# TengdaHan/DPC

Measured on AMD Instinct MI355X. Metric: clips/sec (train step, B x8x3x5xHxW), higher is better.
Workload: dtype bf16; 1 GPU; cfg2: resnet18 2d3d, img_dim 128, seq_len 5, num_seq 8, pred_step 3, batch 128/GPU, full train step (fwd+CE/top-k+bwd+all-reduce+Adam); global_batch=128, parallelism=dp1, init=reference init, random, launch=hipGraph replay, streams=2

## Files before the change

### dpc_amd/csrc/conv_wgrad_patch.hip

```cpp
#include "conv_common.h"
#include <stdlib.h>

struct WgradPatchParams {
    const void* src;
    const void* dy;
    float* part;
    int Co, Ci, dy_ld, src_ld, Kp;
    int RH, W, NF;
    int M;
    int nks, kcps;
    int ntm, ntc;
    unsigned src_bytes, dy_bytes;
    FastDiv d_cpf;
    int cpf;
    int KT, pt, T;
    FastDiv d_T;
    int dbg;
};
#ifdef DPC_WS_PROBE
#define WP_DBG(bit) (p.dbg & (bit))
#else
#define WP_DBG(bit) 0
#endif

template <int RW>
__global__ __launch_bounds__(256, 2) void wgrad_patch_kernel(WgradPatchParams p) {
    constexpr int ROWS = 64 / RW;
    constexpr int PR = ROWS + 2, PW = RW + 4;
    constexpr int NPOS = PR * PW;
    constexpr int NPB = (NPOS + 7) / 8;
    constexpr int NIB = (NPB + 3) / 4;
    constexpr int STAGE = 8192 + NPB * 1024;
    constexpr int NST = (RW == 32 && 2 * 3 * STAGE <= 160 * 1024) ? 3 : 2;
    __shared__ __attribute__((aligned(1024))) unsigned char lds[NST * STAGE];

    const int tid = threadIdx.x;
    const int lane = tid & 63;
#ifdef DPC_SIMT_EMU
    const int wv = tid >> 6;
#else
    const int wv = __builtin_amdgcn_readfirstlane(tid >> 6);
#endif
    const int wi = wv >> 1, wj = wv & 1;
    const int l31 = lane & 31, lhi = lane >> 5;
    int id = blockIdx.x;
    {
        const int nwg = gridDim.x, q = nwg >> 3, r = nwg & 7, x = id & 7;
        id = (x < r ? x * (q + 1) : r * (q + 1) + (x - r) * q) + (id >> 3);
    }
    const int tile_c = id % p.ntc; id /= p.ntc;
    const int tile_m = id % p.ntm; id /= p.ntm;
    const int kt = id % p.KT;
    const int ks = id / p.KT;
    const int nchunks = p.NF * p.cpf;
    const int c_begin = ks * p.kcps;
    const int c_end = (c_begin + p.kcps < nchunks) ? c_begin + p.kcps : nchunks;

    const BufRsrc rs_a = make_buf_rsrc(p.dy, p.dy_bytes);
    const BufRsrc rs_b = make_buf_rsrc(p.src, p.src_bytes);
    const int pl = lane >> 3;
    const int lslot = (lane & 7) ^ (2 * (pl & 3));
    unsigned a_off[2];
    int a_row[2];
    DPC_UNROLL
    for (int i = 0; i < 2; ++i) {
        const int pp = 8 * (wv + 4 * i) + pl;
        const int r = pp / RW, c = pp % RW;
        a_row[i] = c < p.W ? r : (1 << 28);
        a_off[i] = (unsigned)((r * p.W + c) * p.dy_ld + tile_m * 64 + lslot * 8) * 2u;
    }
    unsigned b_off[NIB];
    int b_row[NIB];
    DPC_UNROLL
    for (int i = 0; i < NIB; ++i) {
        const int pp = 8 * (wv + 4 * i) + pl;
        const int prow = pp / PW, pcol = pp % PW;
        const bool ok = pp < NPOS && pcol >= 1 && pcol <= p.W;
        b_row[i] = ok ? prow - 1 : (1 << 28);
        b_off[i] = (unsigned)(((prow - 1) * p.W + (pcol - 1)) * p.src_ld + tile_c * 64 + lslot * 8) * 2u;
    }

    f32x16 acc[9];
    DPC_UNROLL
    for (int t = 0; t < 9; ++t)
        DPC_UNROLL
        for (int r = 0; r < 16; ++r) acc[t][r] = 0.f;

    constexpr int NPC = 2 + NIB;
    unsigned dma_v[NPC];
    unsigned char* dma_stage = lds;
    auto dma_prep = [&](int chunk, int buf, bool real) {
        dma_stage = lds + buf * STAGE;
        const unsigned frame = fdiv((unsigned)chunk, p.d_cpf);
        const int h0 = (chunk - (int)frame * p.cpf) * ROWS;
        const unsigned a_base = (unsigned)(((int)frame * p.RH + h0) * p.W) * (unsigned)p.dy_ld * 2u;
        const unsigned b_base = (unsigned)((((int)frame + kt - p.pt) * p.RH + h0) * p.W) * (unsigned)p.src_ld * 2u;
        DPC_UNROLL
        for (int i = 0; i < 2; ++i) {
            const bool ok = (unsigned)(h0 + a_row[i]) < (unsigned)p.RH;
            dma_v[i] = ok && real ? a_base + a_off[i] : DPC_BUF_OOB;
        }
        DPC_UNROLL
        for (int i = 0; i < NIB; ++i) {
            const bool ok = (unsigned)(h0 + b_row[i]) < (unsigned)p.RH;
            dma_v[2 + i] = ok && real ? b_base + b_off[i] : DPC_BUF_OOB;
        }
    };
    auto dma_piece = [&](auto Ic) {
        constexpr int I = decltype(Ic)::value;
        if (WP_DBG(1)) return;
        if constexpr (I < 2) {
            glds16_buf(rs_a, dma_v[I], 0u, dma_stage + (wv + 4 * I) * 1024, lane);
        } else {
            if constexpr (4 * (I - 2) + 3 < NPB) {
                glds16_buf(rs_b, dma_v[I], 0u, dma_stage + 8192 + (wv + 4 * (I - 2)) * 1024, lane);
            } else {
                if (wv + 4 * (I - 2) < NPB) glds16_buf(rs_b, dma_v[I], 0u, dma_stage + 8192 + (wv + 4 * (I - 2)) * 1024, lane);
            }
        }
    };
    auto issue = [&](int chunk, int buf) {
        dma_prep(chunk, buf, true);
        static_for<NPC>([&](auto Ic) { dma_piece(Ic); });
    };

    const int gq = lane >> 4, s16 = lane & 15, ph = s16 >> 2;
    const int lin = ((gq >> 1) * 8 + ph) * 128;
    auto slot_off = [&](int c0, int phase) {
        const int colb = (c0 + (gq & 1) * 16 + 4 * (s16 & 3)) * 2;
        return ((((colb >> 4) ^ (2 * (phase & 3))) & 7) << 4) + (colb & 15);
    };
    const int fa = lin + slot_off(wi * 32, ph);
    const int linb = ((((gq >> 1) * 8) / RW) * PW + ((gq >> 1) * 8) % RW + ph) * 128;
    int fb[3];
    DPC_UNROLL
    for (int kw = 0; kw < 3; ++kw) fb[kw] = 8192 + linb + slot_off(wj * 32, ph + kw);

#ifdef DPC_SIMT_EMU
    auto compute = [&](int buf) {
        static_for<NPC>([&](auto Ic) { dma_piece(Ic); });
        const unsigned char* st = lds + buf * STAGE;
        DPC_UNROLL
        for (int kk = 0; kk < 4; ++kk) {
            const u32x2 a0 = lds_read_tr16(st + fa + (kk * 16) * 128);
            const u32x2 a1 = lds_read_tr16(st + fa + (kk * 16 + 4) * 128);
            const u32x4 av = {a0[0], a0[1], a1[0], a1[1]};
            const int r = (kk * 16) / RW, w0 = (kk * 16) % RW;
            DPC_UNROLL
            for (int kh = 0; kh < 3; ++kh)
                DPC_UNROLL
                for (int kw = 0; kw < 3; ++kw) {
                    const int pos = (r + kh) * PW + w0 + kw;
                    const u32x2 b0 = lds_read_tr16(st + fb[kw] + pos * 128);
                    const u32x2 b1 = lds_read_tr16(st + fb[kw] + (pos + 4) * 128);
                    const u32x4 bv = {b0[0], b0[1], b1[0], b1[1]};
                    acc[kh * 3 + kw] = mfma_32x32x16_bf16(av, bv, acc[kh * 3 + kw]);
                }
        }
    };
#else
    constexpr int LOOKAHEAD = 4, RB = 8;
    const uint32_t lds0 = (uint32_t)(uintptr_t)(__attribute__((address_space(3))) unsigned char*)lds;
    auto compute = [&](int buf) {
        const uint32_t sa = lds0 + buf * STAGE + fa;
        uint32_t sb[3];
        DPC_UNROLL
        for (int kw = 0; kw < 3; ++kw) sb[kw] = lds0 + buf * STAGE + fb[kw];
        u32x2 alo[2], ahi[2], blo[RB], bhi[RB];
        auto load = [&](auto Ic) {
            constexpr int I = decltype(Ic)::value;
            constexpr int kk = I / 10, r10 = I % 10;
            if constexpr (r10 == 0) {
                asm volatile("ds_read_b64_tr_b16 %0, %1 offset:%2" : "=v"(alo[kk & 1]) : "v"(sa), "n"((kk * 16) * 128) : "memory");
                __builtin_amdgcn_sched_barrier(0);
                asm volatile("ds_read_b64_tr_b16 %0, %1 offset:%2" : "=v"(ahi[kk & 1]) : "v"(sa), "n"((kk * 16 + 4) * 128) : "memory");
                __builtin_amdgcn_sched_barrier(0);
            } else {
                constexpr int tap = r10 - 1, kh = tap / 3, kw = tap % 3, j = 9 * kk + tap;
                constexpr int pos = ((kk * 16) / RW + kh) * PW + (kk * 16) % RW + kw;
                asm volatile("ds_read_b64_tr_b16 %0, %1 offset:%2" : "=v"(blo[j % RB]) : "v"(sb[kw]), "n"(pos * 128) : "memory");
                __builtin_amdgcn_sched_barrier(0);
                asm volatile("ds_read_b64_tr_b16 %0, %1 offset:%2" : "=v"(bhi[j % RB]) : "v"(sb[kw]), "n"((pos + 4) * 128) : "memory");
                __builtin_amdgcn_sched_barrier(0);
            }
        };
        __builtin_amdgcn_sched_barrier(0);
        static_for<36>([&](auto Mc) {
            constexpr int m = decltype(Mc)::value;
            constexpr int kk = m / 9, tap = m % 9, idx = 10 * kk + 1 + tap;
            constexpr int f_prev = m == 0 ? 0 : ((idx - 1 + (tap == 0 ? -1 : 0)) + 1 + LOOKAHEAD < 40 ? (idx - 1 + (tap == 0 ? -1 : 0)) + 1 + LOOKAHEAD : 40);
            constexpr int f_now = idx + 1 + LOOKAHEAD < 40 ? idx + 1 + LOOKAHEAD : 40;
            static_for<f_now - f_prev>([&](auto Dc) { load(std::integral_constant<int, f_prev + decltype(Dc)::value>{}); });
            asm volatile("s_waitcnt lgkmcnt(%0)" ::"n"(2 * (f_now - idx - 1)) : "memory");
            __builtin_amdgcn_sched_barrier(0);
            const u32x4 av = {alo[kk & 1][0], alo[kk & 1][1], ahi[kk & 1][0], ahi[kk & 1][1]};
            const u32x4 bv = {blo[m % RB][0], blo[m % RB][1], bhi[m % RB][0], bhi[m % RB][1]};
            acc[tap] = mfma_32x32x16_bf16(av, bv, acc[tap]);
            __builtin_amdgcn_sched_barrier(0);
            if constexpr (m % 4 == 1 && m / 4 < NPC) {
                dma_piece(std::integral_constant<int, m / 4>{});
                __builtin_amdgcn_sched_barrier(0);
            }
        });
    };
#endif

    auto next_valid = [&](int c) {
        if (p.KT == 1) return c;
        while (c < c_end) {
            const unsigned frame = fdiv((unsigned)c, p.d_cpf);
            const int t = (int)frame - (int)fdiv(frame, p.d_T) * p.T;
            if ((unsigned)(t + kt - p.pt) < (unsigned)p.T) break;
            ++c;
        }
        return c;
    };
    int n_mine = 2;
    DPC_UNROLL
    for (int i = 0; i < NIB; ++i) n_mine += (wv + 4 * i < NPB) ? 1 : 0;
    int cur = next_valid(c_begin), buf = 0;
    if (NST == 3) {
        int nxt = c_end;
        if (cur < c_end) {
            issue(cur, 0);
            nxt = next_valid(cur + 1);
            if (nxt < c_end) issue(nxt, 1);
        }
        while (cur < c_end) {
            if (nxt < c_end) wait_vmcnt_upto(n_mine); else wait_vmcnt<0>();
            if (!WP_DBG(4)) barrier_lds_only();
            const int nxt2 = nxt < c_end ? next_valid(nxt + 1) : c_end;
            dma_prep(nxt2 < c_end ? nxt2 : cur, buf >= 1 ? buf - 1 : 2, nxt2 < c_end);
            if (!WP_DBG(2)) compute(buf);
            else static_for<NPC>([&](auto Ic) { dma_piece(Ic); });
            cur = nxt;
            nxt = nxt2;
            buf = buf == 2 ? 0 : buf + 1;
        }
    } else {
        if (cur < c_end) issue(cur, 0);
        __syncthreads();
        while (cur < c_end) {
            const int nxt = next_valid(cur + 1);
            dma_prep(nxt < c_end ? nxt : cur, buf ^ 1, nxt < c_end);
            if (!WP_DBG(2)) compute(buf);
            else static_for<NPC>([&](auto Ic) { dma_piece(Ic); });
            __syncthreads();
            cur = nxt;
            buf ^= 1;
        }
    }

    const int ci = tile_c * 64 + wj * 32 + l31;
    DPC_UNROLL
    for (int t = 0; t < 9; ++t)
        DPC_UNROLL
        for (int r = 0; r < 16; ++r) {
            const int co = tile_m * 64 + wi * 32 + (r & 3) + 8 * (r >> 2) + 4 * lhi;
            p.part[((long long)ks * p.Co + co) * p.Kp + (kt * 9 + t) * p.Ci + ci] = acc[t][r];
        }
}

static int wgrad_patch_enabled() {
    static int v = -1;
    if (v < 0) {
        const char* e = getenv("DPC_WGRAD_PATCH");
        v = (e && e[0] == '0') ? 0 : 1;
    }
    return v;
}

int dpc_wgrad_patch_try(const dpc_conv_desc* d, const void* src, const void* dy, int dy_ld, float* part, int32_t* nsplit,
                        hipStream_t stream) {
    if (!wgrad_patch_enabled()) return 1;
    if (d->dtype_in != DPC_BF16 || d->mode != 0) return 1;
    if (d->KH != 3 || d->KW != 3 || d->st != 1 || d->sh != 1 || d->sw != 1 || d->ph != 1 || d->pw != 1) return 1;
    if (!((d->KT == 1 && d->pt == 0) || (d->KT == 3 && d->pt == 1))) return 1;
    if (d->RT != d->ST || d->RH != d->SH || d->RW != d->SW) return 1;
    if (d->RW > 64) return 1;
    if (d->Ci % 64 || d->Co % 64 || d->src_ld % 8 || dy_ld % 8 || dy_ld < d->Co) return 1;
    const int rwp = d->RW <= 8 ? 8 : d->RW <= 16 ? 16 : d->RW <= 32 ? 32 : 64;
    const int rows = 64 / rwp;
    if (d->RH * d->RW * 10 < ((d->RH + rows - 1) / rows) * 64 * 6) return 1;
    const long long M = (long long)d->N * d->RT * d->RH * d->RW;
    const long long sb = M * d->src_ld * 2, db = M * dy_ld * 2;
    if (sb >= (1ll << 31) || db >= (1ll << 31)) return 1;
    WgradPatchParams p;
    p.Co = d->Co; p.Ci = d->Ci; p.dy_ld = dy_ld; p.src_ld = d->src_ld; p.Kp = 9 * d->KT * d->Ci;
    p.KT = d->KT; p.pt = d->pt; p.T = d->RT; p.d_T = make_fastdiv((uint32_t)d->RT);
    p.RH = d->RH; p.W = d->RW; p.NF = d->N * d->RT; p.M = (int)M;
    p.ntm = d->Co / 64; p.ntc = d->Ci / 64;
    p.src_bytes = (unsigned)sb; p.dy_bytes = (unsigned)db;
    p.cpf = (d->RH + rows - 1) / rows;
    p.d_cpf = make_fastdiv((uint32_t)p.cpf);
    const int nchunks = p.NF * p.cpf;
    static const int target_blocks = getenv("DPC_WGRAD_PATCH_BLOCKS") ? atoi(getenv("DPC_WGRAD_PATCH_BLOCKS")) : 512;
    int want = target_blocks / (p.ntm * p.ntc * p.KT);
    if (want < 1) want = 1;
    if (want > nchunks) want = nchunks;
    p.kcps = (nchunks + want - 1) / want;
    p.nks = (nchunks + p.kcps - 1) / p.kcps;
    if (nsplit) *nsplit = p.nks;
    if (!part) return DPC_OK;
    if (!src || !dy) return DPC_ERR_ARG;
    if (((uintptr_t)src % 16) || ((uintptr_t)dy % 16)) return DPC_ERR_UNSUPPORTED;
    p.src = src; p.dy = dy; p.part = part;
#ifdef DPC_WS_PROBE
    p.dbg = getenv("DPC_WS_DBG") ? atoi(getenv("DPC_WS_DBG")) : 0;
#else
    p.dbg = 0;
#endif
    dim3 grid((unsigned)(p.ntm * p.ntc * p.KT * p.nks)), block(256);
    if (rwp == 64) {
        DPC_LAUNCH((wgrad_patch_kernel<64>), grid, block, stream, p);
    } else if (rwp == 32) {
        DPC_LAUNCH((wgrad_patch_kernel<32>), grid, block, stream, p);
    } else if (rwp == 8) {
        DPC_LAUNCH((wgrad_patch_kernel<8>), grid, block, stream, p);
    } else {
        DPC_LAUNCH((wgrad_patch_kernel<16>), grid, block, stream, p);
    }
    return dpc_launch_status();
}
```

Before: 5023 clips/s.

## Repartition wgrad patch MFMA work across waves by tap to cut LDS B reads

Each wave previously owned one 32-row Co half and all nine taps, so every wave read all nine B tap fragments from LDS per k-step. Now a wave pair splits the taps: each wave loads both A halves and five B tap slots (the centre tap is shared), reusing each B fragment for two MFMAs. This cuts the LDS transposed reads per MFMA. The block index decode is also reordered so that kt varies fastest, which changes which workgroups run close together and how they share cache. Register pressure rises from holding two A fragments, and the output scatter now maps accumulators to taps through a permutation.

```diff
diff --git a/dpc_amd/csrc/conv_wgrad_patch.hip b/dpc_amd/csrc/conv_wgrad_patch.hip
--- a/dpc_amd/csrc/conv_wgrad_patch.hip
+++ b/dpc_amd/csrc/conv_wgrad_patch.hip
@@ -23,6 +23,11 @@
 #define WP_DBG(bit) 0
 #endif
 
+constexpr int wp_issued(int m, int lookahead, int nop) {
+    const int idx = 7 * (m / 9) + 2 + (m % 9) / 2;
+    return idx + 1 + lookahead < nop ? idx + 1 + lookahead : nop;
+}
+
 template <int RW>
 __global__ __launch_bounds__(256, 2) void wgrad_patch_kernel(WgradPatchParams p) {
     constexpr int ROWS = 64 / RW;
@@ -31,7 +36,11 @@
     constexpr int NPB = (NPOS + 7) / 8;
     constexpr int NIB = (NPB + 3) / 4;
     constexpr int STAGE = 8192 + NPB * 1024;
+#if defined(DPC_WS_PROBE) && defined(DPC_WGP_NST)
+    constexpr int NST = (DPC_WGP_NST == 3 && 2 * 3 * STAGE <= 160 * 1024) ? 3 : 2;
+#else
     constexpr int NST = (RW == 32 && 2 * 3 * STAGE <= 160 * 1024) ? 3 : 2;
+#endif
     __shared__ __attribute__((aligned(1024))) unsigned char lds[NST * STAGE];
 
     const int tid = threadIdx.x;
@@ -41,17 +50,18 @@
 #else
     const int wv = __builtin_amdgcn_readfirstlane(tid >> 6);
 #endif
-    const int wi = wv >> 1, wj = wv & 1;
+    const int h = wv >> 1, wj = wv & 1;
+    auto slot_tap = [&](int s) { return s == 4 ? 4 : 5 * h + s; };
     const int l31 = lane & 31, lhi = lane >> 5;
     int id = blockIdx.x;
     {
         const int nwg = gridDim.x, q = nwg >> 3, r = nwg & 7, x = id & 7;
         id = (x < r ? x * (q + 1) : r * (q + 1) + (x - r) * q) + (id >> 3);
     }
+    const int kt = id % p.KT; id /= p.KT;
     const int tile_c = id % p.ntc; id /= p.ntc;
-    const int tile_m = id % p.ntm; id /= p.ntm;
-    const int kt = id % p.KT;
-    const int ks = id / p.KT;
+    const int tile_m = id % p.ntm;
+    const int ks = id / p.ntm;
     const int nchunks = p.NF * p.cpf;
     const int c_begin = ks * p.kcps;
     const int c_end = (c_begin + p.kcps < nchunks) ? c_begin + p.kcps : nchunks;
@@ -130,11 +140,16 @@
         const int colb = (c0 + (gq & 1) * 16 + 4 * (s16 & 3)) * 2;
         return ((((colb >> 4) ^ (2 * (phase & 3))) & 7) << 4) + (colb & 15);
     };
-    const int fa = lin + slot_off(wi * 32, ph);
+    int fa[2];
+    DPC_UNROLL
+    for (int j = 0; j < 2; ++j) fa[j] = lin + slot_off((h ^ j) * 32, ph);
     const int linb = ((((gq >> 1) * 8) / RW) * PW + ((gq >> 1) * 8) % RW + ph) * 128;
-    int fb[3];
-    DPC_UNROLL
-    for (int kw = 0; kw < 3; ++kw) fb[kw] = 8192 + linb + slot_off(wj * 32, ph + kw);
+    int fb[5];
+    DPC_UNROLL
+    for (int s = 0; s < 5; ++s) {
+        const int tap = slot_tap(s), kh = tap / 3, kw = tap - 3 * kh;
+        fb[s] = 8192 + linb + slot_off(wj * 32, ph + kw) + (kh * PW + kw) * 128;
+    }
 
 #ifdef DPC_SIMT_EMU
     auto compute = [&](int buf) {
@@ -142,60 +157,64 @@
         const unsigned char* st = lds + buf * STAGE;
         DPC_UNROLL
         for (int kk = 0; kk < 4; ++kk) {
-            const u32x2 a0 = lds_read_tr16(st + fa + (kk * 16) * 128);
-            const u32x2 a1 = lds_read_tr16(st + fa + (kk * 16 + 4) * 128);
-            const u32x4 av = {a0[0], a0[1], a1[0], a1[1]};
-            const int r = (kk * 16) / RW, w0 = (kk * 16) % RW;
+            u32x4 av[2];
             DPC_UNROLL
-            for (int kh = 0; kh < 3; ++kh)
-                DPC_UNROLL
-                for (int kw = 0; kw < 3; ++kw) {
-                    const int pos = (r + kh) * PW + w0 + kw;
-                    const u32x2 b0 = lds_read_tr16(st + fb[kw] + pos * 128);
-                    const u32x2 b1 = lds_read_tr16(st + fb[kw] + (pos + 4) * 128);
-                    const u32x4 bv = {b0[0], b0[1], b1[0], b1[1]};
-                    acc[kh * 3 + kw] = mfma_32x32x16_bf16(av, bv, acc[kh * 3 + kw]);
-                }
-        }
-    };
-#else
-    constexpr int LOOKAHEAD = 4, RB = 8;
+            for (int j = 0; j < 2; ++j) {
+                const u32x2 a0 = lds_read_tr16(st + fa[j] + (kk * 16) * 128);
+                const u32x2 a1 = lds_read_tr16(st + fa[j] + (kk * 16 + 4) * 128);
+                av[j] = u32x4{a0[0], a0[1], a1[0], a1[1]};
+            }
+            const int pos = ((kk * 16) / RW) * PW + (kk * 16) % RW;
+            DPC_UNROLL
+            for (int s = 0; s < 5; ++s) {
+                const u32x2 b0 = lds_read_tr16(st + fb[s] + pos * 128);
+                const u32x2 b1 = lds_read_tr16(st + fb[s] + (pos + 4) * 128);
+                const u32x4 bv = {b0[0], b0[1], b1[0], b1[1]};
+                acc[2 * s] = mfma_32x32x16_bf16(av[0], bv, acc[2 * s]);
+                if (s < 4) acc[2 * s + 1] = mfma_32x32x16_bf16(av[1], bv, acc[2 * s + 1]);
+            }
+        }
+    };
+#else
+    constexpr int LOOKAHEAD = 4, RB = 5, NOP = 28;
+    static_assert(RB >= LOOKAHEAD + 1 && 2 * LOOKAHEAD <= 15, "B ring / lgkmcnt range");
     const uint32_t lds0 = (uint32_t)(uintptr_t)(__attribute__((address_space(3))) unsigned char*)lds;
     auto compute = [&](int buf) {
-        const uint32_t sa = lds0 + buf * STAGE + fa;
-        uint32_t sb[3];
-        DPC_UNROLL
-        for (int kw = 0; kw < 3; ++kw) sb[kw] = lds0 + buf * STAGE + fb[kw];
-        u32x2 alo[2], ahi[2], blo[RB], bhi[RB];
+        uint32_t sa[2], sb[5];
+        DPC_UNROLL
+        for (int j = 0; j < 2; ++j) sa[j] = lds0 + buf * STAGE + fa[j];
+        DPC_UNROLL
+        for (int s = 0; s < 5; ++s) sb[s] = lds0 + buf * STAGE + fb[s];
+        u32x2 alo[2][2], ahi[2][2], blo[RB], bhi[RB];
         auto load = [&](auto Ic) {
             constexpr int I = decltype(Ic)::value;
-            constexpr int kk = I / 10, r10 = I % 10;
-            if constexpr (r10 == 0) {
-                asm volatile("ds_read_b64_tr_b16 %0, %1 offset:%2" : "=v"(alo[kk & 1]) : "v"(sa), "n"((kk * 16) * 128) : "memory");
-                __builtin_amdgcn_sched_barrier(0);
-                asm volatile("ds_read_b64_tr_b16 %0, %1 offset:%2" : "=v"(ahi[kk & 1]) : "v"(sa), "n"((kk * 16 + 4) * 128) : "memory");
+            constexpr int kk = I / 7, r7 = I % 7;
+            if constexpr (r7 < 2) {
+                asm volatile("ds_read_b64_tr_b16 %0, %1 offset:%2" : "=v"(alo[kk & 1][r7]) : "v"(sa[r7]), "n"((kk * 16) * 128) : "memory");
+                __builtin_amdgcn_sched_barrier(0);
+                asm volatile("ds_read_b64_tr_b16 %0, %1 offset:%2" : "=v"(ahi[kk & 1][r7]) : "v"(sa[r7]), "n"((kk * 16 + 4) * 128) : "memory");
                 __builtin_amdgcn_sched_barrier(0);
             } else {
-                constexpr int tap = r10 - 1, kh = tap / 3, kw = tap % 3, j = 9 * kk + tap;
-                constexpr int pos = ((kk * 16) / RW + kh) * PW + (kk * 16) % RW + kw;
-                asm volatile("ds_read_b64_tr_b16 %0, %1 offset:%2" : "=v"(blo[j % RB]) : "v"(sb[kw]), "n"(pos * 128) : "memory");
-                __builtin_amdgcn_sched_barrier(0);
-                asm volatile("ds_read_b64_tr_b16 %0, %1 offset:%2" : "=v"(bhi[j % RB]) : "v"(sb[kw]), "n"((pos + 4) * 128) : "memory");
+                constexpr int s = r7 - 2, j = 5 * kk + s;
+                constexpr int pos = ((kk * 16) / RW) * PW + (kk * 16) % RW;
+                asm volatile("ds_read_b64_tr_b16 %0, %1 offset:%2" : "=v"(blo[j % RB]) : "v"(sb[s]), "n"(pos * 128) : "memory");
+                __builtin_amdgcn_sched_barrier(0);
+                asm volatile("ds_read_b64_tr_b16 %0, %1 offset:%2" : "=v"(bhi[j % RB]) : "v"(sb[s]), "n"((pos + 4) * 128) : "memory");
                 __builtin_amdgcn_sched_barrier(0);
             }
         };
         __builtin_amdgcn_sched_barrier(0);
         static_for<36>([&](auto Mc) {
             constexpr int m = decltype(Mc)::value;
-            constexpr int kk = m / 9, tap = m % 9, idx = 10 * kk + 1 + tap;
-            constexpr int f_prev = m == 0 ? 0 : ((idx - 1 + (tap == 0 ? -1 : 0)) + 1 + LOOKAHEAD < 40 ? (idx - 1 + (tap == 0 ? -1 : 0)) + 1 + LOOKAHEAD : 40);
-            constexpr int f_now = idx + 1 + LOOKAHEAD < 40 ? idx + 1 + LOOKAHEAD : 40;
+            constexpr int kk = m / 9, t = m % 9, s = t / 2, co = t & 1, idx = 7 * kk + 2 + s, j = 5 * kk + s;
+            constexpr int f_prev = m == 0 ? 0 : wp_issued(m - 1, LOOKAHEAD, NOP);
+            constexpr int f_now = wp_issued(m, LOOKAHEAD, NOP);
             static_for<f_now - f_prev>([&](auto Dc) { load(std::integral_constant<int, f_prev + decltype(Dc)::value>{}); });
             asm volatile("s_waitcnt lgkmcnt(%0)" ::"n"(2 * (f_now - idx - 1)) : "memory");
             __builtin_amdgcn_sched_barrier(0);
-            const u32x4 av = {alo[kk & 1][0], alo[kk & 1][1], ahi[kk & 1][0], ahi[kk & 1][1]};
-            const u32x4 bv = {blo[m % RB][0], blo[m % RB][1], bhi[m % RB][0], bhi[m % RB][1]};
-            acc[tap] = mfma_32x32x16_bf16(av, bv, acc[tap]);
+            const u32x4 av = {alo[kk & 1][co][0], alo[kk & 1][co][1], ahi[kk & 1][co][0], ahi[kk & 1][co][1]};
+            const u32x4 bv = {blo[j % RB][0], blo[j % RB][1], bhi[j % RB][0], bhi[j % RB][1]};
+            acc[t] = mfma_32x32x16_bf16(av, bv, acc[t]);
             __builtin_amdgcn_sched_barrier(0);
             if constexpr (m % 4 == 1 && m / 4 < NPC) {
                 dma_piece(std::integral_constant<int, m / 4>{});
@@ -253,12 +272,14 @@
 
     const int ci = tile_c * 64 + wj * 32 + l31;
     DPC_UNROLL
-    for (int t = 0; t < 9; ++t)
+    for (int t = 0; t < 9; ++t) {
+        const int tap = slot_tap(t >> 1), cb = tile_m * 64 + (h ^ (t & 1)) * 32 + 4 * lhi;
         DPC_UNROLL
         for (int r = 0; r < 16; ++r) {
-            const int co = tile_m * 64 + wi * 32 + (r & 3) + 8 * (r >> 2) + 4 * lhi;
-            p.part[((long long)ks * p.Co + co) * p.Kp + (kt * 9 + t) * p.Ci + ci] = acc[t][r];
-        }
+            const int co = cb + (r & 3) + 8 * (r >> 2);
+            p.part[((long long)ks * p.Co + co) * p.Kp + (kt * 9 + tap) * p.Ci + ci] = acc[t][r];
+        }
+    }
 }
 
 static int wgrad_patch_enabled() {
```

Result: no change. 5022 clips/s (-0.0%).
